# RobustFieldAutonomyLab/DRL_graph_exploration

Hardware: AMD Instinct MI355X
Metric: env-steps/sec (256 parallel envs, ~64-node graphs) (higher is better)
Workload: dtype f64; 1 GPU; configs[1]: 256 envs/GPU, 40x40 map (V=1600), 100 landmarks, belief update at ~59-node graphs (P=37.0 poses, L=22.2 landmarks, M=188 factors) from a device snapshot; envs_per_gpu=256, map_size=40, num_landmarks=100, parallelism=env-sharded x1

## Files before the change

### drl_graph_exploration_amd/csrc/drlgx_dev.h

```cpp
#pragma once
#include <hip/hip_runtime.h>
#include <stdint.h>

#include "../../include/drlgx.h"
#include "map_carve.h"

#define DRLGX_MT_N 624
#define DRLGX_MT_STRIDE 626
#define DRLGX_CNT_STRIDE 8
#define DRLGX_RED_STRIDE 8
#define DRLGX_PRIOR_STRIDE 16

enum { C_P = 0, C_L = 1, C_M = 2, C_STEP = 3, C_ISAM = 4, C_NEWP = 5, C_NEWL = 6, C_FLAG = 7 };
enum { R_UTR = 0, R_KNOWN = 1, R_EXPL = 2, R_UDET = 3, R_UWTR = 4, R_DIST = 5, R_OBS = 6, R_LATCH = 7 };

struct DrlgxState {
  drlgx_config cfg;
  int n_envs, n_inst, n_roll;
  int P_max, L_max, M_max, LG, V, Vu, rows, cols, A_max;
  int win;
  int disc_cells;
  int count_explored;
  double lo_free, lo_occ, lo_min, lo_max, occ_thresh;
  int bbox_noop;
// ... 76 lines not shown
#define DRLGX_KS_REF (*(const DrlgxState *)S_)
#define DRLGX_KS_ARG(S) ((DrlgxStateConst)(S).self_dev)

#define DRLGX_PROF(S, slot)                                                        \
  do {                                                                             \
    if ((S).prof && threadIdx.x == 0 && blockIdx.x == (S).prof_block) (S).prof[slot] = wall_clock64(); \
  } while (0)

__device__ __forceinline__ int drlgx_bid() {
  int b = blockIdx.x;
  asm volatile("" : "+v"(b));
  return __builtin_amdgcn_readfirstlane(b);
}

__device__ __forceinline__ int drlgx_tid() {
  int t = threadIdx.x;
  asm volatile("" : "+v"(t));
  return t;
}

struct LaunchSel {
  int base;
  int n;
  const uint8_t *active;
  const int32_t *n_act;
  int act_idx;
  int map_last_only = 0;
  int pcap = 0;
  int skip_map = 0;
  const unsigned char *simlog = nullptr;
  size_t simlog_roll = 0;
  int simlog_act = 0;
  int vm_from = -1;
  __host__ __device__ __forceinline__ int cap(int P_max) const { return pcap > 0 && pcap < P_max ? pcap : P_max; }
  __device__ __forceinline__ bool map_on(int i) const {
    return !(map_last_only && n_act) || act_idx == n_act[i] - 1;
  }
  __device__ __forceinline__ bool on(int i) const {
    if (active && !active[i]) return false;
    if (n_act && act_idx >= n_act[i]) return false;
    return true;
  }
};

struct Pose {
  double x, y, c, s;
};
struct P2 {
  double x, y;
};

__device__ __forceinline__ void rot_from_cos_sin(double c, double s, double &oc, double &os) {
  if (fabs(c * c + s * s - 1.0) > 1e-9) {
    double n = sqrt(c * c + s * s);
    c /= n;
    s /= n;
  }
  oc = c;
  os = s;
}
__device__ __forceinline__ Pose make_pose(double x, double y, double th) { return Pose{x, y, cos(th), sin(th)}; }
__device__ __forceinline__ double theta_of(const Pose &p) { return atan2(p.s, p.c); }
__device__ __forceinline__ Pose compose(const Pose &a, const Pose &b) {
  Pose r;
  rot_from_cos_sin(a.c * b.c - a.s * b.s, a.s * b.c + a.c * b.s, r.c, r.s);
  r.x = a.x + (a.c * b.x - a.s * b.y);
// ... 492 lines not shown
```

### drl_graph_exploration_amd/csrc/drlgx_engine.cpp

```cpp
#include <hip/hip_runtime.h>

#include <algorithm>
#include <chrono>
#include <cmath>
#include <cstdio>
#include <cstring>
#include <functional>
#include <string>
#include <unordered_map>
#include <cstdlib>
#include <vector>

#include "drlgx_dev.h"
#include "drlgx_fields.h"

#define HIPCHK(e, call)                                                                       \
  do {                                                                                        \
    hipError_t _r = (call);                                                                   \
    if (_r != hipSuccess) {                                                                   \
      (e)->last_error = std::string(#call) + ": " + hipGetErrorString(_r);                    \
      return DRLGX_E_HIP;                                                                     \
    }                                                                                         \
  } while (0)

// ... 39 lines not shown
  bool la_loop = true;
  double *fm2_sig = nullptr, *fm2_scratch = nullptr;
  int *fm2_iscratch = nullptr;
  int32_t *fm2_slot = nullptr;
  size_t fm2_sig_stride = 0, fm2_scratch_stride = 0;
  double *em_cov = nullptr;
  int32_t *em_nout = nullptr;
  int *em_flag = nullptr;
  int *og_flag = nullptr;
  double *tree_act = nullptr, *tree_cand_act = nullptr, *tree_cost = nullptr;
  int *tree_link = nullptr, *tree_leaf = nullptr, *tree_meta = nullptr;
  int32_t *tree_cand_env = nullptr, *tree_cand_n = nullptr;
  size_t tree_nodes_cap = 0, tree_sel_cap = 0, tree_cand_cap = 0;
  double sampler_max_nodes = 0.5, sampler_safe_distance = 0.0;
  int sampler_dubins = 0;
  int sampler_obstacles = 0;
  int env_obstacles = 0;
  double *follow_act = nullptr;
  int dubins_leaf_scoring = 0;
  uint8_t *tree_cand_core = nullptr;
  double *tree_cand_dist = nullptr;
  size_t tree_cand_steps_cap = 0, tree_cand_last = 0;
  bool tree_cand_last_steps = false;
  DrlgxDubins dubins = {};
  double *dub_end_x = nullptr, *dub_end_y = nullptr, *dub_v = nullptr, *dub_w = nullptr, *tree_pose = nullptr;
  int *dub_steps = nullptr;
  size_t dub_cap = 0, tree_pose_cap = 0;
  double dub_reach = 0.0;
  int dub_prefilter = 1;
  std::vector<double> dub_end_h, dub_v_h, dub_w_h;
  std::vector<int> dub_steps_h;
  int owed_slot = -1;
  bool restore_eager = false;
};

#define DRLGX_ENTER_OWING(e)                    \
  do {                                          \
    if (e) {                                    \
      (void)hipSetDevice((e)->device);          \
      state_sync(e);                            \
    }                                           \
  } while (0)
#define DRLGX_ENTER(e)                          \
  do {                                          \
    DRLGX_ENTER_OWING(e);                       \
    if (e) settle(e);                           \
  } while (0)

struct drlgx_engine;
static void state_sync(drlgx_engine *e);
static void settle(drlgx_engine *e);

namespace {

template <typename T>
int dev_alloc(drlgx_engine *e, T **out, size_t count) {
  void *p = nullptr;
  size_t bytes = std::max<size_t>(count * sizeof(T), 256);
  HIPCHK(e, hipMalloc(&p, bytes));
  HIPCHK(e, hipMemsetAsync(p, 0, bytes, e->stream));
  e->allocs.push_back(p);
  *out = reinterpret_cast<T *>(p);
  return DRLGX_OK;
}

template <typename T>
// ... 59 lines not shown
      cfg->max_actions < 1 || cfg->num_samples < 1)
    return DRLGX_E_INVALID;
  if (!(cfg->resolution >= 1)) {
    g_create_error = "resolution must be at least 1";
    return DRLGX_E_INVALID;
  }
  if (cfg->max_poses > 65535 || cfg->max_landmarks > 65535 || cfg->max_factors > 65534) return DRLGX_E_INVALID;
  if (!drlgx_slam_capacity_ok(cfg->max_poses, cfg->max_landmarks, cfg->max_factors)) return DRLGX_E_INVALID;
  const double cells = std::floor((cfg->map_max_x - cfg->map_min_x) / cfg->resolution) *
                       std::floor((cfg->map_max_y - cfg->map_min_y) / cfg->resolution);
  if (!(cells <= 65535.0) || !drlgx_graph_capacity_ok(cfg->max_poses, cfg->max_landmarks, (int)cells)) {
    g_create_error = "max_landmarks x max_poses (or the cell count of the map) too large for the LDS tables of the graph export";
    return DRLGX_E_INVALID;
  }
  if (kmap::MapCarve(cfg->max_poses, 1, (int)cells, false).bytes > kmap::kLdsBudget) {
    g_create_error = "map too large for the LDS tables of the map kernel";
    return DRLGX_E_INVALID;
  }
  return DRLGX_OK;
}

static bool env_flag(const char *name, bool dflt) {
  const char *v = getenv(name);
  if (!v) return dflt;
  return dflt ? v[0] != '0' : v[0] == '1';
}

static void read_env_switches(drlgx_engine *e) {
  e->by_capacity = env_flag("DRLGX_VARIANT_BY_CAPACITY", false);
  e->spin_sync = env_flag("DRLGX_SYNC_SPIN", true);
  e->la_presim = env_flag("DRLGX_LOOKAHEAD_PRESIM", true);
  e->la_loop = env_flag("DRLGX_LOOKAHEAD_LOOP", true);
  e->restore_eager = env_flag("DRLGX_RESTORE_EAGER", false);
}

static double p2l(double p) { return std::log(p / (1.0 - p)); }
static double l2p(double l) { return std::exp(l) / (1.0 + std::exp(l)); }

static int disc_cells_bound(double r) {
  const int n = 32;
  const double h = 0.5 / n, rr = r + h * 0.70710678118654752440 + 1e-9;
  const int k = (int)std::ceil(rr) + 1;
  int best = 0;
  for (int a = 0; a < n; ++a)
    for (int b = 0; b < n; ++b) {
      const double u = (a + 0.5) * h, v = (b + 0.5) * h;
      int cnt = 0;
      for (int i = -k; i <= k; ++i)
        for (int j = -k; j <= k; ++j)
          if ((i - u) * (i - u) + (j - v) * (j - v) <= rr * rr) ++cnt;
      best = std::max(best, cnt);
    }
  return best;
}

static int set_map_constants(drlgx_engine *e) {
  DrlgxState &S = e->S;
  const drlgx_config *cfg = &S.cfg;
  S.P_max = cfg->max_poses;
  S.L_max = cfg->max_landmarks;
  S.M_max = cfg->max_factors;
  S.LG = std::max(cfg->num_landmarks, 1);
  S.A_max = cfg->max_actions;
  S.cols = (int)std::floor((cfg->map_max_x - cfg->map_min_x) / cfg->resolution);
  S.rows = (int)std::floor((cfg->map_max_y - cfg->map_min_y) / cfg->resolution);
  S.V = S.rows * S.cols;
// ... 411 lines not shown
  DRLGX_ENTER_OWING(e);
  if (!e || (bytes > 0 && (!src_dev || !dst_host))) return DRLGX_E_INVALID;
  return status_fetch(e, src_dev, bytes, dst_host);
}

int drlgx_reset_host(drlgx_engine *e, int n, const int32_t *env_ids, const uint32_t *seeds, const double *start) {
  DRLGX_ENTER(e);
  if (!e || n <= 0 || n > e->S.n_envs || !env_ids || !seeds || !start) return DRLGX_E_INVALID;
  std::vector<uint8_t> mask(e->S.n_envs, 0);
  for (int i = 0; i < n; ++i) {
    if (env_ids[i] < 0 || env_ids[i] >= e->S.n_envs || mask[env_ids[i]]) return DRLGX_E_INVALID;
    mask[env_ids[i]] = 1;
  }
  HIPCHK(e, hipMemcpyAsync(e->stage_i32, env_ids, n * sizeof(int32_t), hipMemcpyHostToDevice, e->stream));
  HIPCHK(e, hipMemcpyAsync(e->stage_u32, seeds, n * sizeof(uint32_t), hipMemcpyHostToDevice, e->stream));
  HIPCHK(e, hipMemcpyAsync(e->stage_f64, start, n * 3 * sizeof(double), hipMemcpyHostToDevice, e->stream));
  HIPCHK(e, hipMemcpyAsync(e->stage_mask, mask.data(), e->S.n_envs, hipMemcpyHostToDevice, e->stream));
  HIPCHK(e, hipMemsetAsync(e->S.status, 0, sizeof(int), e->stream));
  drlgx_launch_reset(e->S, e->stream, n, e->stage_i32, e->stage_u32, e->stage_f64);
  for (int i = 0; i < n; ++i) e->pbound[env_ids[i]] = 1;
  LaunchSel sel{0, e->S.n_envs, e->stage_mask, nullptr, 0};
  drlgx_launch_slam(e->S, e->stream, sel, e->by_capacity ? e->S.P_max : 1);
  sel.pcap = max_bound(e);
  drlgx_launch_map(e->S, e->stream, sel, 0);
  int r = check_launch(e);
  if (r) return r;
  HIPCHK(e, hipStreamSynchronize(e->stream));
  return DRLGX_OK;
}

static void launch_belief_step(drlgx_engine *e, LaunchSel sel, const double *odom, int odom_stride, int n_measure, int pb, bool may_split,
                               bool obstacles = false) {
  const DrlgxState &S = e->S;
  sel.pcap = pb;
  if (drlgx_step_fusable(S, pb) && !e->per_stage && !obstacles) {
    ScopedTimer t(e, 5);
    const bool split = may_split && sel.n > e->n_cu && drlgx_map_two_per_cu(S, pb);
    sel.skip_map = split ? 1 : 0;
    drlgx_launch_step(S, e->stream, sel, odom, odom_stride, n_measure);
    if (split) {
      sel.skip_map = 0;
      drlgx_launch_map(S, e->stream, sel, 1);
    }
  } else if (drlgx_step_arrow_fusable(S) && !e->per_stage && !obstacles) {
    ScopedTimer t(e, 5);
    drlgx_launch_step_arrow(S, e->stream, sel, odom, odom_stride, n_measure);
  } else {
    {
      ScopedTimer t(e, 0);
      if (obstacles) drlgx_launch_sim_obs(S, e->stream, sel, odom, odom_stride);
      else drlgx_launch_sim(S, e->stream, sel, odom, odom_stride, n_measure);
    }
    {
      ScopedTimer t(e, 1);
      drlgx_launch_slam(S, e->stream, sel, pb);
    }
    {
      ScopedTimer t(e, 2);
      drlgx_launch_map(S, e->stream, sel, 1);
    }
  }
}

static bool env_obstacles_on(const drlgx_engine *e) { return e->env_obstacles && e->S.cfg.safe_distance > 0.0; }

int drlgx_step(drlgx_engine *e, const double *odom_dev, const uint8_t *active_dev) {
// ... 11 lines not shown
  return check_launch(e);
}

int drlgx_step_plan(drlgx_engine *e, const double *actions_dev, const int32_t *n_actions_dev, int action_index, int map_last_only) {
  DRLGX_ENTER(e);
  if (!e || !actions_dev || !n_actions_dev || action_index < 0 || action_index >= e->S.A_max) return DRLGX_E_INVALID;
  LaunchSel sel{0, e->S.n_envs, nullptr, n_actions_dev, action_index};
  sel.map_last_only = map_last_only ? 1 : 0;
  const int pb = std::min(max_bound(e) + 1, e->S.P_max);
  advance_pbound(e, 1);
  launch_belief_step(e, sel, actions_dev, e->S.A_max * 3, 2, pb, false, env_obstacles_on(e));
  return check_launch(e);
}

static void presimulate(drlgx_engine *e, LaunchSel &sel, const double *act, int n_measure, int max_n_actions) {
  const DrlgxState &S = e->S;
  const size_t entry = drlgx_simlog_entry_bytes(S), roll = entry * (size_t)S.A_max;
  if (!e->simlog_dev && dev_alloc(e, &e->simlog_dev, roll * (size_t)S.n_roll) != DRLGX_OK) {
    (void)hipGetLastError();
    e->last_error.clear();
    e->la_presim = false;
    return;
  }
  ScopedTimer t(e, 0);
  drlgx_launch_presim(S, e->stream, sel, act, S.A_max * 3, n_measure, max_n_actions, e->simlog_dev, roll, (int)entry);
  sel.simlog = e->simlog_dev;
  sel.simlog_roll = roll;
  sel.simlog_act = (int)entry;
}

static int launch_action_range(drlgx_engine *e, LaunchSel sel, const double *act, int n_measure, int pbe, int max_n_actions, bool partial,
                               bool presim) {
  const DrlgxState &S = e->S;
  int a_sw = 0;
  while (a_sw < max_n_actions && drlgx_step_fusable(S, std::min(pbe + a_sw + 1, S.P_max))) ++a_sw;
  const bool rest_loops = a_sw == max_n_actions || drlgx_step_arrow_fusable(S);
  if (!e->la_loop || e->per_stage || !(rest_loops || (partial && a_sw > 0))) return 0;
  if (presim && e->la_presim && rest_loops) presimulate(e, sel, act, n_measure, max_n_actions);
  ScopedTimer t(e, 5);
  if (a_sw > 0) {
    sel.act_idx = 0;
    sel.pcap = std::min(pbe + 1, S.P_max);
    drlgx_launch_step_loop(S, e->stream, sel, act, S.A_max * 3, n_measure, a_sw);
  }
  if (a_sw == max_n_actions || !rest_loops) return a_sw;
  sel.act_idx = a_sw;
  sel.pcap = std::min(pbe + a_sw + 1, S.P_max);
  drlgx_launch_step_arrow_loop(S, e->stream, sel, act, S.A_max * 3, n_measure, max_n_actions);
  return max_n_actions;
}

int drlgx_step_plans(drlgx_engine *e, const double *actions_dev, const int32_t *n_actions_dev, int max_n_actions, int map_last_only) {
  DRLGX_ENTER(e);
  if (!e || !actions_dev || !n_actions_dev || max_n_actions < 0 || max_n_actions > e->S.A_max) return DRLGX_E_INVALID;
  if (max_n_actions == 0) return DRLGX_OK;
  LaunchSel sel{0, e->S.n_envs, nullptr, n_actions_dev, 0};
  sel.map_last_only = map_last_only ? 1 : 0;
  const int a_begin = env_obstacles_on(e) ? 0 : launch_action_range(e, sel, actions_dev, 2, max_bound(e), max_n_actions, false, false);
  advance_pbound(e, a_begin);
  for (int a = a_begin; a < max_n_actions; ++a) {
    const int r = drlgx_step_plan(e, actions_dev, n_actions_dev, a, map_last_only);
    if (r) return r;
  }
  return check_launch(e);
}

// ... 58 lines not shown
  HIPCHK(e, hipMemsetAsync(e->S.status, 0, sizeof(int), e->stream));
  drlgx_launch_reset(e->S, e->stream, n, e->stage_i32, e->stage_u32, e->stage_f64, 0);
  for (int i = 0; i < n; ++i) e->pbound[env_ids[i]] = 1;
  int r = check_launch(e);
  if (r) return r;
  HIPCHK(e, hipStreamSynchronize(e->stream));
  return DRLGX_OK;
}
int drlgx_stage_move(drlgx_engine *e, const double *odom_dev, const uint8_t *active_dev) {
  DRLGX_ENTER(e);
  if (!e || !odom_dev) return DRLGX_E_INVALID;
  advance_pbound(e, 1);
  drlgx_launch_sim_stage(e->S, e->stream, LaunchSel{0, e->S.n_envs, active_dev, nullptr, 0}, odom_dev, 0, nullptr, nullptr, nullptr);
  return check_launch(e);
}
int drlgx_stage_measure(drlgx_engine *e, const uint8_t *active_dev, int32_t *keys_dev, double *bearing_range_dev, int32_t *count_dev) {
  DRLGX_ENTER(e);
  if (!e || !keys_dev || !bearing_range_dev || !count_dev) return DRLGX_E_INVALID;
  HIPCHK(e, hipMemsetAsync(count_dev, 0, sizeof(int32_t) * e->S.n_envs, e->stream));
  drlgx_launch_sim_stage(e->S, e->stream, LaunchSel{0, e->S.n_envs, active_dev, nullptr, 0}, nullptr, 1, keys_dev, bearing_range_dev,
                         count_dev);
  return check_launch(e);
}
int drlgx_stage_add_measurements(drlgx_engine *e, const uint8_t *active_dev, const int32_t *keys_dev, const double *bearing_range_dev,
                                 const int32_t *count_dev) {
  DRLGX_ENTER(e);
  if (!e || !keys_dev || !bearing_range_dev || !count_dev) return DRLGX_E_INVALID;
  drlgx_launch_add_measurements(e->S, e->stream, LaunchSel{0, e->S.n_envs, active_dev, nullptr, 0}, keys_dev, bearing_range_dev, count_dev);
  return check_launch(e);
}
int drlgx_stage_optimize(drlgx_engine *e, const uint8_t *active_dev) {
  DRLGX_ENTER(e);
  if (!e) return DRLGX_E_INVALID;
  drlgx_launch_slam(e->S, e->stream, LaunchSel{0, e->S.n_envs, active_dev, nullptr, 0}, max_bound(e));
  return check_launch(e);
}
int drlgx_stage_update_map(drlgx_engine *e, const uint8_t *active_dev, int rebuild) {
  DRLGX_ENTER(e);
  if (!e) return DRLGX_E_INVALID;
  drlgx_launch_map(e->S, e->stream, LaunchSel{0, e->S.n_envs, active_dev, nullptr, 0}, rebuild ? 1 : 0);
  return check_launch(e);
}

static const int kFm2Chunk = 128, kFm2MaxMeas = 256;
static int fm2_run(drlgx_engine *e, int n_cand, const int32_t *cand_env_dev, const double *actions_dev, const int32_t *n_actions_dev,
                   const uint8_t *core_dev, double *cov_out, int out_stride_poses, int32_t *n_out, bool chunk_out, const std::function<void(int, int)> &after) {
  const DrlgxState &S = e->S;
  if (!e->fm2_sig) {
    const size_t nmax = (size_t)3 * S.P_max + 2 * S.L_max;
    e->fm2_sig_stride = nmax * nmax;
    e->fm2_scratch_stride = drlgx_fm2_scratch_doubles(S, kFm2MaxMeas);
    int r;
    if ((r = dev_alloc(e, &e->fm2_sig, e->fm2_sig_stride * (size_t)S.n_envs))) return r;
    if ((r = dev_alloc(e, &e->fm2_scratch, e->fm2_scratch_stride * (size_t)kFm2Chunk))) return r;
    if ((r = dev_alloc(e, &e->fm2_iscratch, (size_t)2 * kFm2MaxMeas * kFm2Chunk))) return r;
    if ((r = dev_alloc(e, &e->fm2_slot, (size_t)S.n_envs))) return r;
    std::vector<int32_t> ident(S.n_envs);
    for (int i = 0; i < S.n_envs; ++i) ident[i] = i;
    HIPCHK(e, hipMemcpyAsync(e->fm2_slot, ident.data(), ident.size() * sizeof(int32_t), hipMemcpyHostToDevice, e->stream));
    HIPCHK(e, hipStreamSynchronize(e->stream));
  }
  drlgx_launch_fm2_prior(S, e->stream, nullptr, S.n_envs, e->fm2_sig, e->fm2_sig_stride, 3 * S.P_max + 2 * S.L_max);
  for (int c0 = 0; c0 < n_cand; c0 += kFm2Chunk) {
    const int nc = std::min(kFm2Chunk, n_cand - c0);
    drlgx_launch_fm2_update(S, e->stream, 0, nc, cand_env_dev + c0, e->fm2_slot, actions_dev + (size_t)c0 * S.A_max * 3, n_actions_dev + c0,
                            core_dev ? core_dev + (size_t)c0 * S.A_max : nullptr, e->fm2_sig, e->fm2_sig_stride, e->fm2_scratch, e->fm2_scratch_stride, e->fm2_iscratch, kFm2MaxMeas,
                            chunk_out ? cov_out : cov_out + (size_t)c0 * out_stride_poses * 9, out_stride_poses,
// ... 869 lines not shown
```

### drl_graph_exploration_amd/csrc/k_inc.hip

```cpp

#pragma once
#include <type_traits>
#include "k_slam_common.hip"
namespace kslam {
#pragma clang fp contract(on)

constexpr int IYS = 18;
constexpr int INF = 64;
constexpr int kStreamKB = 512;
constexpr int ISNT = 4;

__device__ __forceinline__ int *inc_meta(const DrlgxState &S, int inst) { return S.jc_meta + (size_t)inst * 4; }

__device__ __forceinline__ bool inc_precheck(const DrlgxState &S, int inst, int P_after, int tid, int *scratch, int meta0 = -1, int meta1 = 0,
                                             int isam = 0) {
  if (!S.jc) return false;
  const int *meta = inc_meta(S, inst);
  const int *cnt = S.cnt + (size_t)inst * DRLGX_CNT_STRIDE;
  if (meta0 < 0) {
    meta0 = meta[0];
    meta1 = meta[1];
    isam = cnt[C_ISAM];
  }
  if (meta0 != 1 || meta1 + 1 != P_after || P_after < 2) return false;
// ... 72 lines not shown
  x.fq = reinterpret_cast<double *>(take(32 * 8));
  x.recs = reinterpret_cast<double *>(take(INF * REC * 8));
  x.gs = reinterpret_cast<double *>(take(INEW * 12 * 8));
  x.vvec = reinterpret_cast<double *>(take(32 * 8));
  x.wks = reinterpret_cast<double *>(take(5 * 16 * IYS * 8));
  x.thp = reinterpret_cast<double *>(take((size_t)P * 4 * 8));
  x.thl = reinterpret_cast<double *>(take((size_t)x.Lcap * 2 * 8));
  x.dl = reinterpret_cast<double *>(take((size_t)ncap * 8));
  x.Dl = reinterpret_cast<double *>(take((size_t)P * 6 * 8));
  x.Y = reinterpret_cast<double *>(take((size_t)(x.n1p + 1) * IYS * 8));
  x.cwl = reinterpret_cast<double *>(smem_raw + off);
  const size_t fixed = ((plan_off + 15) & ~(size_t)15) + (off - off0);
  if (fixed > (size_t)lds_bytes) return false;
  lds_panel = fixed + (size_t)ncap * x.ldw * 8 <= (size_t)lds_bytes;
  const size_t pan = lds_panel ? (size_t)ncap * x.ldw * 8 : 0, yh = (size_t)(x.n1p + 1) * IYS * 8;
  x.Yh = x.cwl + pan / 8;
  x.wide = fixed + pan + yh <= (size_t)lds_bytes;
  x.snt = 0;
  if (!lds_panel && (3 * P + 1 + 15) / 16 > kDenseTiles) {
    x.yrows = x.a0 + 1;
    const size_t y_off = (size_t)(reinterpret_cast<unsigned char *>(x.Y) - smem_raw);
    const size_t avail = (size_t)lds_bytes - (((plan_off + 15) & ~(size_t)15) + (y_off - off0));
    for (int t = ISNT; t >= 1 && !x.snt; --t)
      if ((size_t)t * x.yrows * IYS * 8 + (size_t)max(0, t * t - 5) * 16 * IYS * 8 + (size_t)16 * t * 8 * 8 + 64 * 8 <= avail) x.snt = t;
    x.yt = x.Y;
    x.wim = x.yt + (size_t)x.snt * x.yrows * IYS;
    x.jt = x.wim + (size_t)max(0, x.snt * x.snt - 5) * 16 * IYS;
    x.svv = x.jt + (size_t)16 * x.snt * 8;
  }
  return true;
}

template <bool kLds, bool kSub>
__device__ __forceinline__ void inc_pre(const DrlgxState &S, const IncCtx &x, int tid, const double *odom3, SubBarrier sb) {
  const int ft = kSub ? tid - 64 : tid, fn = kSub ? kThreads - 64 : kThreads, lane = tid & 63;
  auto bar = [&]() {
    if constexpr (kSub) sb.sync(lane);
    else __syncthreads();
  };
  const int inst = x.inst, P = x.P, pn = x.pn, pp = x.pp, L0 = x.L0, n1 = x.n1, a0 = x.a0;
  double *gpan = S.jc + (size_t)inst * S.jc_stride;
  auto growp = [&](int q) -> double * { return gpan + (size_t)(q < 3 * P ? q : q + 3 * (S.P_max - P)) * S.jc_ld; };
  auto rowp = [&](int q) -> double * {
    if constexpr (kLds) return x.cwl + (size_t)q * x.ldw;
    else return gpan + (size_t)(q < 3 * P ? q : q + 3 * (S.P_max - P)) * S.jc_ld;
  };
  const double *th_pose = S.th_pose + (size_t)inst * S.P_max * 4;
  const double *th_lm = S.th_lm + (size_t)inst * S.L_max * 2;
  const double *d_pose = S.d_pose + (size_t)inst * S.P_max * 3;
  const double *d_lm = S.d_lm + (size_t)inst * S.L_max * 2;
  const double *jd = S.jd + (size_t)inst * S.P_max * 6;
  if (S.prof && blockIdx.x == S.prof_block && ft == 0) S.prof[0] = wall_clock64();
  if (ft < 4) x.ictl[ft] = 0;
  if (ft == fn - 1) {
    const double *t1 = th_pose + 4 * pp;
    Pose p1{t1[0], t1[1], t1[2], t1[3]}, p2, om;
    if constexpr (kSub) {
      om = make_pose(odom3[0], odom3[1], odom3[2]);
      const double *ep = S.est_pose + ((size_t)inst * S.P_max + pp) * 4;
      p2 = compose(Pose{ep[0], ep[1], ep[2], ep[3]}, om);
    } else {
      const double *t2 = th_pose + 4 * pn, *oo = S.odo + ((size_t)inst * S.P_max + pp) * 4;
      p2 = Pose{t2[0], t2[1], t2[2], t2[3]};
      om = Pose{oo[0], oo[1], oo[2], oo[3]};
    }
    double H1[9];
    const Pose hx = between(p1, p2, H1);
// ... 19 lines not shown
        const int q0 = qq, q1 = qq + rs, q2 = qq + 2 * rs, q3 = qq + 3 * rs;
        auto src = [&](int q) { const int c = min(q, nr - 1); return reinterpret_cast<const double2 *>(growp(c < 3 * pn ? c : c + 3))[cp]; };
        const double2 v0 = src(q0), v1 = src(q1), v2 = src(q2), v3 = src(q3);
        auto dst = [&](int q, const double2 &v) { if (q < nr) reinterpret_cast<double2 *>(rowp(q < 3 * pn ? q : q + 3))[cp] = v; };
        dst(q0, v0); dst(q1, v1); dst(q2, v2); dst(q3, v3);
      }
  }
  for (int e = ft; e < (x.n1p + 1 - n1) * IYS; e += fn) {
    x.Y[(size_t)n1 * IYS + e] = 0.0;
    if (x.wide) x.Yh[(size_t)n1 * IYS + e] = 0.0;
  }
  bar();
  if (S.prof && blockIdx.x == S.prof_block && ft == 0) S.prof[1] = wall_clock64();
  const double *fq = x.fq;
  {
    const double f00 = fq[0], f01 = fq[1], f02 = fq[2], f10 = fq[3], f11 = fq[4], f12 = fq[5], f20 = fq[6], f21 = fq[7], f22 = fq[8];
    for (int qq = ft; qq < n1 - 3; qq += fn) {
      const int q = qq < 3 * pn ? qq : qq + 3;
      double *r = rowp(q);
      const double t0 = r[0], t1 = r[1], t2 = r[2];
      r[0] = f00 * t0 + f01 * t1 + f02 * t2;
      r[1] = f10 * t0 + f11 * t1 + f12 * t2;
      r[2] = f20 * t0 + f21 * t1 + f22 * t2;
    }
  }
  bar();
  for (int e = ft; e < 3 * a0; e += fn) {
    const int r = e / a0, c = e - r * a0;
    double v = fq[3 * r] * rowp(3 * pp)[c] + fq[3 * r + 1] * rowp(3 * pp + 1)[c] + fq[3 * r + 2] * rowp(3 * pp + 2)[c];
    if (c == r) v += 1.0 / (c < 2 ? S.w_trans : S.w_rot);
    rowp(3 * pn + r)[c] = v;
  }
  if (ft < 3) x.dl[3 * pn + ft] = fq[3 * ft] * x.dl[3 * pp] + fq[3 * ft + 1] * x.dl[3 * pp + 1] + fq[3 * ft + 2] * x.dl[3 * pp + 2] + fq[9 + ft];
  if (S.prof && blockIdx.x == S.prof_block && ft == 0) S.prof[2] = wall_clock64();
}

template <bool kLds, int kSNT = ISNT>
__device__ __forceinline__ bool inc_post(const DrlgxState &S, const IncCtx &x, int L, int M, const SimBox &box, int tid,
                                         double *hand = nullptr, int hand_cap = 0) {
  const int lane = tid & 63, wave = tid >> 6, lc = lane & 15, lr = lane >> 4;
  const int inst = x.inst, P = x.P, pn = x.pn, L0 = x.L0, M0 = x.M0, n1 = x.n1, n1p = x.n1p, a0 = x.a0;
  int *meta = inc_meta(S, inst);
  const int nf = M - M0, nn = L - L0;
  const int n = 3 * P + 2 * L, a = 3 + 2 * L;
  int *fre = x.fre, *fnew = x.fnew, *fslot = x.fslot, *ictl = x.ictl;
  double *recs = x.recs, *gs = x.gs, *vvec = x.vvec, *wks = x.wks, *thp = x.thp, *thl = x.thl, *dl = x.dl, *Dl = x.Dl, *Y = x.Y;
  double *gpan = S.jc + (size_t)inst * S.jc_stride;
  auto growp = [&](int q) -> double * { return gpan + (size_t)(q < 3 * P ? q : q + 3 * (S.P_max - P)) * S.jc_ld; };
  auto rowp = [&](int q) -> double * {
    if constexpr (kLds) return x.cwl + (size_t)q * x.ldw;
    else return gpan + (size_t)(q < 3 * P ? q : q + 3 * (S.P_max - P)) * S.jc_ld;
  };
  int *cnt = S.cnt + (size_t)inst * DRLGX_CNT_STRIDE;
  double *d_pose = S.d_pose + (size_t)inst * S.P_max * 3;
  double *d_lm = S.d_lm + (size_t)inst * S.L_max * 2;
  double *jd = S.jd + (size_t)inst * S.P_max * 6;
  const bool feasible = nf >= 0 && nf <= INF && nn >= 0 && nn <= nf && L <= x.Lcap;
  const int *slot_src = box.br ? box.slot : S.meas_lm + (size_t)inst * S.M_max + M0;
  const double *br_src = box.br ? box.br : S.meas_br + ((size_t)inst * S.M_max + M0) * 2;
  const double *nl_src = box.br ? box.lm : S.th_lm + ((size_t)inst * S.L_max + L0) * 2;
  if (feasible && tid < 64) {
    const bool have = tid < nf;
    const int slot = have ? slot_src[tid] : -1;
    if (have) fslot[tid] = slot;
    bool bad = have && (slot < 0 || slot >= L);
    if (have && !box.br) bad |= S.meas_pose[(size_t)inst * S.M_max + M0 + tid] != pn;
    for (int t = 0; t < nf; ++t) {
      const int st = __builtin_amdgcn_readlane(slot, t);
      bad |= have && t < tid && st == slot;
    }
    const bool re = have && slot < L0, nw = have && slot >= L0;
    const unsigned long long mre = __ballot(re), mnw = __ballot(nw);
    if (re) fre[__popcll(mre & ((1ull << lane) - 1ull))] = tid;
    if (nw && !bad) fnew[slot - L0] = tid;
    if ((__ballot(bad) || __popcll(mnw) != nn) && lane == 0) ictl[2] = 1;
    if (lane == 0) ictl[0] = __popcll(mre);
  }
  for (int e = tid - 64; e >= 0 && e < 2 * nn && feasible; e += kThreads - 64) thl[2 * L0 + e] = nl_src[e];
  __syncthreads();
  if (!feasible || ictl[2]) {
    if (!kLds && tid == 0) meta[0] = 0;
    return false;
  }
  const int n_re = ictl[0];
  if (tid < nf) linearize_br(thp + 4 * pn, thl + 2 * fslot[tid], br_src[2 * tid], br_src[2 * tid + 1], recs + (size_t)REC * tid);
  __syncthreads();
  DRLGX_PROF(S, 35);
  const double Rb = S.cfg.bearing_noise * S.cfg.bearing_noise, Rr = S.cfg.range_noise * S.cfg.range_noise;
  const int ntr = n1p >> 4, ntc = (a0 + 15) >> 4;
  auto batch = [&](int b0, int nb, auto wide_tag) {
    constexpr bool kWide = decltype(wide_tag)::value;
    const int k = 2 * nb, kD = kWide ? k - 16 : 0;
    double *Yh = x.Yh;
    {
      constexpr int FS = kWide ? 16 : 8, RS = kThreads / FS;
      const int f = tid & (FS - 1);
      double j0 = 0, j1 = 0, j2 = 0, j3 = 0, j4 = 0, j5 = 0, l0c = 0, l1c = 0, l2c = 0, l3c = 0;
      int cl = 3;
      if (f < nb) {
        const int t = fre[b0 + f];
        const double *rc = recs + (size_t)REC * t;
        j0 = rc[0]; j1 = rc[1]; j2 = rc[2]; j3 = rc[3]; j4 = rc[4]; j5 = rc[5];
        l0c = rc[6]; l1c = rc[7]; l2c = rc[8]; l3c = rc[9];
        cl = 3 + 2 * fslot[t];
      }
      double *Yf = (kWide && f >= 8) ? Yh : Y;
      const int k0 = ks16(2 * (f & 7)), k1 = ks16(2 * (f & 7) + 1);
      for (int q0 = tid / FS; q0 < n1; q0 += 4 * RS) {
        double c0[4], c1[4], c2[4], l0[4], l1[4];
#pragma unroll
        for (int u = 0; u < 4; ++u) {
          const double *r = rowp(min(q0 + u * RS, n1 - 1));
          c0[u] = r[0]; c1[u] = r[1]; c2[u] = r[2]; l0[u] = r[cl]; l1[u] = r[cl + 1];
        }
#pragma unroll
        for (int u = 0; u < 4; ++u) {
          const int q = q0 + u * RS;
          if (q < n1) {
            Yf[(size_t)q * IYS + k0] = c0[u] * j0 + c1[u] * j1 + c2[u] * j2 + l0[u] * l0c + l1[u] * l1c;
            Yf[(size_t)q * IYS + k1] = c0[u] * j3 + c1[u] * j4 + c2[u] * j5 + l0[u] * l2c + l1[u] * l3c;
          }
        }
      }
    }
    __syncthreads();
    if (b0 == 0) DRLGX_PROF(S, 36);
    if (wave == 0) {
      auto tent = [&](int i, int j) -> double {
        const int t = fre[b0 + (i >> 1)], u = i & 1;
        const double *rc = recs + (size_t)REC * t;
        const double *Yj = (kWide && j >= 16) ? Yh : Y;
        const int col = ks16(j & 15);
        const double *yp = Yj + (size_t)(3 * pn) * IYS + col, *yl = Yj + (size_t)(3 * P + 2 * fslot[t]) * IYS + col;
        double sv = rc[3 * u] * yp[0] + rc[3 * u + 1] * yp[IYS] + rc[3 * u + 2] * yp[2 * IYS] + rc[6 + 2 * u] * yl[0] + rc[7 + 2 * u] * yl[IYS];
        if (i == j) sv += u ? Rr : Rb;
        return sv;
      };
      if (lane < (kWide ? 32 : 16)) {
        double v = 0.0;
        if (lane < k) {
          const int t = fre[b0 + (lane >> 1)], u = lane & 1;
// ... 568 lines not shown
    cnt[C_ISAM] = cnt[C_ISAM] + 1;
    cnt[C_NEWP] = P;
    cnt[C_NEWL] = L;
    if (ictl[1]) atomicMin(S.status, DRLGX_E_NUMERIC);
    if (S.inc_stats) atomicAdd(S.inc_stats, 1ull);
  }
  DRLGX_PROF(S, 7);
  return true;
}

__device__ __forceinline__ void panel_invalidate(const DrlgxState &S, int inst, int tid) {
  if (S.jc && tid == 0) {
    inc_meta(S, inst)[0] = 0;
    if (S.inc_stats) atomicAdd(S.inc_stats + 1, 1ull);
  }
}

#pragma clang fp contract(fast)

template <int kSNT>
__device__ __forceinline__ bool inc_stage(const DrlgxState &S, const LaunchSel &sel, int lds_bytes, size_t smem_off) {
  const int tid = drlgx_tid(), bi = drlgx_bid();
  if (!S.jc || !sel.on(bi)) return false;
  const int inst = sel.base + bi;
  const int *cnt = S.cnt + (size_t)inst * DRLGX_CNT_STRIDE;
  if (cnt[C_FLAG]) return false;
  const int P = cnt[C_P], L = cnt[C_L], M = cnt[C_M];
  extern __shared__ __attribute__((aligned(16))) unsigned char smem_raw[];
  if (!inc_precheck(S, inst, P, tid, reinterpret_cast<int *>(smem_raw + smem_off))) return false;
  IncCtx x;
  bool lds_panel = false;
  if (!inc_plan(S, inst, P, lds_bytes, smem_off, x, lds_panel, sel.cap(S.P_max))) return false;
  const SimBox nobox{nullptr, nullptr, nullptr};
  bool done;
  if (lds_panel) {
    inc_pre<true, false>(S, x, tid, nullptr, SubBarrier{nullptr, 0, 0});
    __syncthreads();
    done = inc_post<true, kSNT>(S, x, L, M, nobox, tid);
  } else {
    inc_pre<false, false>(S, x, tid, nullptr, SubBarrier{nullptr, 0, 0});
    __syncthreads();
    done = inc_post<false, kSNT>(S, x, L, M, nobox, tid);
  }
  if (!done) __syncthreads();
  return done;
}
#pragma clang fp contract(off)
}
```

### drl_graph_exploration_amd/csrc/k_slam_common.hip

```cpp
#pragma once
#include "k_sweep.hip"
#include "arrow_carve.h"
#include "slam_carve.h"
namespace kslam {
#pragma clang fp contract(fast)
constexpr int kLdsBudget = 160 * 1024;
static_assert(kFastTilesArrow == 8, "inc_plan (k_inc.hip) spells the reach of k_step_arrow out as 16 * 8");

constexpr int REC = 12;

#pragma clang fp contract(on)
__device__ __forceinline__ void linearize_br(const double *tp, const double *tl, double bm, double rm, double *rec) {
  Pose ps{tp[0], tp[1], tp[2], tp[3]};
  P2 lm{tl[0], tl[1]};
  const P2 d = transform_to(ps, lm);
  const double d2 = d.x * d.x + d.y * d.y, n = sqrt(d2);
  double sm, cm;
  sincos(bm, &sm, &cm);
  if (n > 1e-5) {
    const double in = 1.0 / n;
    const double c = d.x * in, s = d.y * in;
    const double a = -s * in, b = c * in;
    rec[0] = -a;
    rec[1] = -b;
    rec[2] = a * d.y - b * d.x;
    rec[3] = -c;
    rec[4] = -s;
    rec[5] = 0.0;
    rec[6] = a * ps.c - b * ps.s;
    rec[7] = a * ps.s + b * ps.c;
    rec[8] = ps.c * c - ps.s * s;
    rec[9] = ps.s * c + ps.c * s;
    rec[10] = atan2(-sm * c + cm * s, cm * c + sm * s);
    rec[11] = n - rm;
  } else {
    double Jx[6], Jl[4];
    (void)bearing_of<true>(ps, lm, Jx, Jl);
    const double rp = range_of<true>(ps, lm, Jx + 3, Jl + 2);
    for (int k = 0; k < 6; ++k) rec[k] = Jx[k];
    for (int k = 0; k < 4; ++k) rec[6 + k] = Jl[k];
    rec[10] = atan2(-sm, cm);
    rec[11] = rp - rm;
  }
}

__device__ __forceinline__ size_t up8(size_t b) { return (b + 7) & ~(size_t)7; }

#pragma clang fp contract(fast)
#define FOR_EACH_OBSERVING_POSE(mk, W, p)                                      \
  for (int _w = 0; _w < (W); ++_w)                                            \
    for (unsigned long long _m = (mk)[_w]; _m; _m &= _m - 1)                  \
      if (const int p = 64 * _w + __ffsll((long long)_m) - 1; true)

__device__ __forceinline__ void pose_block(const DrlgxState &S, int inst, const double *thp, const double *odo, const double *rec, const int *mstart,
                                           int i, int P, double wb, double wr, double *B, double *g, double *O) {
  const drlgx_config &cfg = S.cfg;
  for (int k = 0; k < 9; ++k) B[k] = 0.0;
  for (int k = 0; k < 3; ++k) g[k] = 0.0;
  const Pose ti{thp[4 * i], thp[4 * i + 1], thp[4 * i + 2], thp[4 * i + 3]};
  if (i == 0) {
    const double *pr = S.prior + (size_t)inst * DRLGX_PRIOR_STRIDE;
    const Pose h = between(Pose{pr[0], pr[1], pr[2], pr[3]}, ti, nullptr);
    const double e[3] = {h.x, h.y, theta_of(h)};
    const double J[9] = {h.c, h.s, 0, -h.s, h.c, 0, 0, 0, 1};
    const double *W = pr + 4;
    double WJ[9], We[3];
    for (int r = 0; r < 3; ++r) {
      for (int c = 0; c < 3; ++c) WJ[r * 3 + c] = W[r * 3] * J[c] + W[r * 3 + 1] * J[3 + c] + W[r * 3 + 2] * J[6 + c];
      We[r] = W[r * 3] * e[0] + W[r * 3 + 1] * e[1] + W[r * 3 + 2] * e[2];
    }
    for (int r = 0; r < 3; ++r) {
      for (int c = 0; c < 3; ++c) B[r * 3 + c] += J[r] * WJ[c] + J[3 + r] * WJ[3 + c] + J[6 + r] * WJ[6 + c];
      g[r] += J[r] * We[0] + J[3 + r] * We[1] + J[6 + r] * We[2];
    }
  }
  const double wo[3] = {1.0 / (cfg.translation_noise * cfg.translation_noise),
// ... 121 lines not shown
```

### drl_graph_exploration_amd/csrc/k_step.hip

```cpp
#include "drlgx_dev.h"

#include "k_sim.hip"
#include "k_sweep.hip"
#include "k_slam_common.hip"
#include "k_inc.hip"
#include "k_slam.hip"
#include "k_slam_arrow.hip"
#include "k_slam_host.hip"
#include "k_map.hip"
#include "k_em.hip"
#include "k_og.hip"

namespace kstep {

__host__ __device__ inline size_t sim_lds_bytes(int LG, int P_max) { return drlgx_sim_lds_bytes(LG, P_max); }

template <int FT>
__device__ __forceinline__ void step_once(const DrlgxState &S, const LaunchSel &sel, const double *odom, int odom_stride, int n_measure,
                                          int lds_bytes, int map_chunk) {
  static_assert(kslam::kThreads == kmap::kThreads, "the fused kernel runs both stages with one workgroup size");
  extern __shared__ __attribute__((aligned(16))) unsigned char step_smem[];
  const int tid = drlgx_tid();
  const int bi = drlgx_bid();
  if (S.prof && tid == 0 && bi < 448) S.prof[128 + 2 * bi] = wall_clock64();
// ... 23 lines not shown
      pan_L0 = mv.z;
      pan_M0 = mv.w;
    }
    const double *od = odom + (size_t)bi * odom_stride + (size_t)sel.act_idx * 3;
    od3[0] = od[0]; od3[1] = od[1]; od3[2] = od[2];
    if (spre.have) ksim::sim_preload(S, inst, tid, n_measure, spre);
    accepted = ksim::move_accepted(S, od3[0], od3[1], P0);
    inc_try = accepted && kslam::inc_precheck(S, inst, P0 + 1, tid, sub_cnt, meta0, meta1, isam);
    const int Lb = min(S.L_max, L0 + 48), Mb = min(S.M_max, M0 + 48);
    pre = accepted && !inc_try && (3 * (P0 + 1) + 1 + 15) / 16 <= kslam::kDenseTiles && kslam::SlamCtx::big_fits(sim_bytes, lds_bytes, P0 + 1, Lb, Mb);
    if (pre) ctx.setup<true>(S, step_smem, sim_bytes, lds_bytes, inst, P0 + 1, Lb, Mb);
  }
  if (tid == 0) {
    sub_cnt[0] = 0;
    sub_cnt[1] = -1;
  }
  __syncthreads();
  if (tid < 64) {
    uint32_t *l0 = reinterpret_cast<uint32_t *>(step_smem);
    uint32_t *l1 = l0 + DRLGX_MT_STRIDE;
    double *dyn = sim_dyn;
    if (sel.simlog)
      ksim::replay_step_body(S, sel, odom, odom_stride, tid, sub_cnt + 1);
    else
      ksim::sim_step_body(S, sel, odom, odom_stride, n_measure, l0, l1, dyn, tid, nullptr, nullptr, nullptr, true, sub_cnt + 1,
                          n_measure == 2 ? lmbox : nullptr, sel.on(bi) ? P0 : -1, L0, M0, spre);
  } else if (pre) {
    ctx.front<true>(S, tid, P0, L0, M0, P0, L0, isam + 1, false, od3, kslam::SubBarrier{sub_cnt, kslam::kThreads / 64 - 1, 0});
  } else if (inc_try) {
    kslam::IncCtx ix;
    bool inc_lds = false;
    if (kslam::inc_plan(S, sel.base + bi, P0 + 1, lds_bytes, sim_bytes, ix, inc_lds, pc, pan_L0, pan_M0)) {
      const kslam::SubBarrier sb{sub_cnt, kslam::kThreads / 64 - 1, 0};
      if (inc_lds) kslam::inc_pre<true, true>(S, ix, tid, od3, sb);
      else kslam::inc_pre<false, true>(S, ix, tid, od3, sb);
    }
  }
  __syncthreads();
  DRLGX_PROF(S, 32);
  if (accepted && tid >= 64 && !sel.simlog) {
    uint32_t *g = S.mt + (size_t)(sel.base + bi) * 2 * DRLGX_MT_STRIDE;
    const uint32_t *img = reinterpret_cast<const uint32_t *>(step_smem);
    for (int i = tid - 64; i < 2 * DRLGX_MT_STRIDE; i += kslam::kThreads - 64) g[i] = img[i];
  }
  const kmap::MapCarve map_carve(pc, map_chunk, S.V, false);
  const bool hand = map_carve.stage + 16 <= sim_bytes - 16;
  const double *lm_lds = nullptr;
  bool inc_done = false;
  if (inc_try) {
    kslam::IncCtx ix;
    bool inc_lds = false;
    if (kslam::inc_plan(S, sel.base + bi, P0 + 1, lds_bytes, sim_bytes, ix, inc_lds, pc, pan_L0, pan_M0)) {
      double *hp = hand ? reinterpret_cast<double *>(step_smem) : nullptr;
      inc_done = inc_lds ? kslam::inc_post<true, 0>(S, ix, sub_cnt[2], sub_cnt[3], box, tid, hp, pc)
                         : kslam::inc_post<false, 0>(S, ix, sub_cnt[2], sub_cnt[3], box, tid, hp, pc);
      if (inc_done) lm_lds = ix.thl;
      else __syncthreads();
    }
  }
  if (!inc_done)
    kslam::slam_finish<FT>(S, sel, lds_bytes, sim_bytes, ctx, pre, sub_cnt + 1, hand ? reinterpret_cast<double *>(step_smem) : nullptr, &lm_lds, box, pc);
  __syncthreads();
  const bool handed = hand && lm_lds != nullptr;
  if (sel.on(bi)) {
    const bool appended = sub_cnt[1] >= 0;
    lo.P = appended ? sub_cnt[1] : P0;
    lo.L = appended ? sub_cnt[2] : L0;
    lo.flag = appended ? 0 : 1;
  }
  const unsigned char *map_masks = step_smem + map_carve.mask;
  if (!handed || reinterpret_cast<const unsigned char *>(lm_lds + 2 * (size_t)S.L_max) > map_masks) lm_lds = nullptr;
  if (!sel.skip_map) kmap::map_body<false>(S, sel, 1, map_chunk, handed, lm_lds, lo);
  if (S.prof && tid == 0 && bi < 448) S.prof[129 + 2 * bi] = wall_clock64();
}

template <int FT>
__global__ __launch_bounds__(kslam::kThreads) void k_step(DrlgxState S, LaunchSel sel, const double *odom, int odom_stride,
                                                          int n_measure, int lds_bytes, int map_chunk) {
  step_once<FT>(S, sel, odom, odom_stride, n_measure, lds_bytes, map_chunk);
}

template <int FT>
__global__ __launch_bounds__(kslam::kThreads) void k_step_ref(DrlgxStateConst Sp, LaunchSel sel, const double *odom, int odom_stride,
                                                              int n_measure, int lds_bytes, int map_chunk) {
  if (__builtin_amdgcn_readfirstlane((int)threadIdx.x >> 6) == 0) drlgx_warm_state(Sp);
  step_once<FT>(*(const DrlgxState *)Sp, sel, odom, odom_stride, n_measure, lds_bytes, map_chunk);
}

// ... 98 lines not shown
```

Before: 4.051 million env-steps/sec.

## Pre-linearize landmark bearing-range Jacobians during the incremental-SLAM pre-phase

Splits bearing-range linearization into a Jacobian part and a measurement-error part. While the simulator waves run, the SLAM waves in inc_pre now compute the Jacobians for all existing landmarks into a scratch buffer. inc_post then copies those precomputed records and only linearizes new landmarks, with one wave computing the error terms while the others start the panel accumulation. This shortens the critical path after the sim phase, at the cost of extra linearization work for landmarks that may not be re-observed and more branching and scratch traffic.

After: 4.079 million env-steps/sec (median of 6 runs). About the same (+0.7%).

```diff
diff --git a/drl_graph_exploration_amd/csrc/drlgx_dev.h b/drl_graph_exploration_amd/csrc/drlgx_dev.h
--- a/drl_graph_exploration_amd/csrc/drlgx_dev.h
+++ b/drl_graph_exploration_amd/csrc/drlgx_dev.h
@@ -132,6 +132,7 @@
   size_t simlog_roll = 0;
   int simlog_act = 0;
   int vm_from = -1;
+  int inc_prelin = 0;
   __host__ __device__ __forceinline__ int cap(int P_max) const { return pcap > 0 && pcap < P_max ? pcap : P_max; }
   __device__ __forceinline__ bool map_on(int i) const {
     return !(map_last_only && n_act) || act_idx == n_act[i] - 1;
diff --git a/drl_graph_exploration_amd/csrc/drlgx_engine.cpp b/drl_graph_exploration_amd/csrc/drlgx_engine.cpp
--- a/drl_graph_exploration_amd/csrc/drlgx_engine.cpp
+++ b/drl_graph_exploration_amd/csrc/drlgx_engine.cpp
@@ -95,6 +95,7 @@
   std::vector<int> dub_steps_h;
   int owed_slot = -1;
   bool restore_eager = false;
+  bool inc_prelin = true;
 };
 
 #define DRLGX_ENTER_OWING(e)                    \
@@ -220,6 +221,7 @@
   e->la_presim = env_flag("DRLGX_LOOKAHEAD_PRESIM", true);
   e->la_loop = env_flag("DRLGX_LOOKAHEAD_LOOP", true);
   e->restore_eager = env_flag("DRLGX_RESTORE_EAGER", false);
+  e->inc_prelin = env_flag("DRLGX_INC_PRELIN", true);
 }
 
 static double p2l(double p) { return std::log(p / (1.0 - p)); }
@@ -697,6 +699,7 @@
 static void launch_belief_step(drlgx_engine *e, LaunchSel sel, const double *odom, int odom_stride, int n_measure, int pb, bool may_split,
                                bool obstacles = false) {
   const DrlgxState &S = e->S;
+  sel.inc_prelin = e->inc_prelin ? 1 : 0;
   sel.pcap = pb;
   if (drlgx_step_fusable(S, pb) && !e->per_stage && !obstacles) {
     ScopedTimer t(e, 5);
@@ -774,6 +777,7 @@
 static int launch_action_range(drlgx_engine *e, LaunchSel sel, const double *act, int n_measure, int pbe, int max_n_actions, bool partial,
                                bool presim) {
   const DrlgxState &S = e->S;
+  sel.inc_prelin = e->inc_prelin ? 1 : 0;
   int a_sw = 0;
   while (a_sw < max_n_actions && drlgx_step_fusable(S, std::min(pbe + a_sw + 1, S.P_max))) ++a_sw;
   const bool rest_loops = a_sw == max_n_actions || drlgx_step_arrow_fusable(S);
@@ -898,7 +902,9 @@
 int drlgx_stage_optimize(drlgx_engine *e, const uint8_t *active_dev) {
   DRLGX_ENTER(e);
   if (!e) return DRLGX_E_INVALID;
-  drlgx_launch_slam(e->S, e->stream, LaunchSel{0, e->S.n_envs, active_dev, nullptr, 0}, max_bound(e));
+  LaunchSel sel{0, e->S.n_envs, active_dev, nullptr, 0};
+  sel.inc_prelin = e->inc_prelin ? 1 : 0;
+  drlgx_launch_slam(e->S, e->stream, sel, max_bound(e));
   return check_launch(e);
 }
 int drlgx_stage_update_map(drlgx_engine *e, const uint8_t *active_dev, int rebuild) {
diff --git a/drl_graph_exploration_amd/csrc/k_inc.hip b/drl_graph_exploration_amd/csrc/k_inc.hip
--- a/drl_graph_exploration_amd/csrc/k_inc.hip
+++ b/drl_graph_exploration_amd/csrc/k_inc.hip
@@ -128,7 +128,7 @@
 }
 
 template <bool kLds, bool kSub>
-__device__ __forceinline__ void inc_pre(const DrlgxState &S, const IncCtx &x, int tid, const double *odom3, SubBarrier sb) {
+__device__ __forceinline__ void inc_pre(const DrlgxState &S, const IncCtx &x, int tid, const double *odom3, SubBarrier sb, bool prelin) {
   const int ft = kSub ? tid - 64 : tid, fn = kSub ? kThreads - 64 : kThreads, lane = tid & 63;
   auto bar = [&]() {
     if constexpr (kSub) sb.sync(lane);
@@ -214,11 +214,13 @@
     rowp(3 * pn + r)[c] = v;
   }
   if (ft < 3) x.dl[3 * pn + ft] = fq[3 * ft] * x.dl[3 * pp] + fq[3 * ft + 1] * x.dl[3 * pp + 1] + fq[3 * ft + 2] * x.dl[3 * pp + 2] + fq[9 + ft];
+  if (prelin)
+    for (int j = ft; j < L0; j += fn) linearize_br_jac(x.thp + 4 * pn, x.thl + 2 * j, x.Y + (size_t)REC * j);
   if (S.prof && blockIdx.x == S.prof_block && ft == 0) S.prof[2] = wall_clock64();
 }
 
 template <bool kLds, int kSNT = ISNT>
-__device__ __forceinline__ bool inc_post(const DrlgxState &S, const IncCtx &x, int L, int M, const SimBox &box, int tid,
+__device__ __forceinline__ bool inc_post(const DrlgxState &S, const IncCtx &x, int L, int M, const SimBox &box, int tid, bool prelin,
                                          double *hand = nullptr, int hand_cap = 0) {
   const int lane = tid & 63, wave = tid >> 6, lc = lane & 15, lr = lane >> 4;
   const int inst = x.inst, P = x.P, pn = x.pn, L0 = x.L0, M0 = x.M0, n1 = x.n1, n1p = x.n1p, a0 = x.a0;
@@ -265,7 +267,16 @@
     return false;
   }
   const int n_re = ictl[0];
-  if (tid < nf) linearize_br(thp + 4 * pn, thl + 2 * fslot[tid], br_src[2 * tid], br_src[2 * tid + 1], recs + (size_t)REC * tid);
+  if (prelin) {
+    for (int e = tid; e < REC * n_re; e += kThreads) {
+      const int i = e / REC, t = fre[i];
+      recs[(size_t)REC * t + (e - REC * i)] = Y[(size_t)REC * fslot[t] + (e - REC * i)];
+    }
+    const int t = kThreads - 1 - tid;
+    if (t < nf && fslot[t] >= L0) linearize_br(thp + 4 * pn, thl + 2 * fslot[t], br_src[2 * t], br_src[2 * t + 1], recs + (size_t)REC * t);
+  } else if (tid < nf) {
+    linearize_br(thp + 4 * pn, thl + 2 * fslot[tid], br_src[2 * tid], br_src[2 * tid + 1], recs + (size_t)REC * tid);
+  }
   __syncthreads();
   DRLGX_PROF(S, 35);
   const double Rb = S.cfg.bearing_noise * S.cfg.bearing_noise, Rr = S.cfg.range_noise * S.cfg.range_noise;
@@ -274,8 +285,15 @@
     constexpr bool kWide = decltype(wide_tag)::value;
     const int k = 2 * nb, kD = kWide ? k - 16 : 0;
     double *Yh = x.Yh;
-    {
-      constexpr int FS = kWide ? 16 : 8, RS = kThreads / FS;
+    const bool spare = prelin && b0 == 0;
+    if (spare && wave == 0) {
+      if (lane < n_re) {
+        const int t = fre[lane];
+        linearize_br_err(recs + (size_t)REC * t, br_src[2 * t], br_src[2 * t + 1]);
+      }
+    } else {
+      constexpr int FS = kWide ? 16 : 8;
+      const int RS = (spare ? kThreads - 64 : kThreads) / FS, rt = spare ? tid - 64 : tid;
       const int f = tid & (FS - 1);
       double j0 = 0, j1 = 0, j2 = 0, j3 = 0, j4 = 0, j5 = 0, l0c = 0, l1c = 0, l2c = 0, l3c = 0;
       int cl = 3;
@@ -288,7 +306,7 @@
       }
       double *Yf = (kWide && f >= 8) ? Yh : Y;
       const int k0 = ks16(2 * (f & 7)), k1 = ks16(2 * (f & 7) + 1);
-      for (int q0 = tid / FS; q0 < n1; q0 += 4 * RS) {
+      for (int q0 = rt / FS; q0 < n1; q0 += 4 * RS) {
         double c0[4], c1[4], c2[4], l0[4], l1[4];
 #pragma unroll
         for (int u = 0; u < 4; ++u) {
@@ -923,15 +941,16 @@
   bool lds_panel = false;
   if (!inc_plan(S, inst, P, lds_bytes, smem_off, x, lds_panel, sel.cap(S.P_max))) return false;
   const SimBox nobox{nullptr, nullptr, nullptr};
+  const bool prelin = kSNT == 0 && sel.inc_prelin != 0;
   bool done;
   if (lds_panel) {
-    inc_pre<true, false>(S, x, tid, nullptr, SubBarrier{nullptr, 0, 0});
-    __syncthreads();
-    done = inc_post<true, kSNT>(S, x, L, M, nobox, tid);
+    inc_pre<true, false>(S, x, tid, nullptr, SubBarrier{nullptr, 0, 0}, prelin);
+    __syncthreads();
+    done = inc_post<true, kSNT>(S, x, L, M, nobox, tid, prelin);
   } else {
-    inc_pre<false, false>(S, x, tid, nullptr, SubBarrier{nullptr, 0, 0});
-    __syncthreads();
-    done = inc_post<false, kSNT>(S, x, L, M, nobox, tid);
+    inc_pre<false, false>(S, x, tid, nullptr, SubBarrier{nullptr, 0, 0}, prelin);
+    __syncthreads();
+    done = inc_post<false, kSNT>(S, x, L, M, nobox, tid, prelin);
   }
   if (!done) __syncthreads();
   return done;
diff --git a/drl_graph_exploration_amd/csrc/k_slam_common.hip b/drl_graph_exploration_amd/csrc/k_slam_common.hip
--- a/drl_graph_exploration_amd/csrc/k_slam_common.hip
+++ b/drl_graph_exploration_amd/csrc/k_slam_common.hip
@@ -10,13 +10,11 @@
 constexpr int REC = 12;
 
 #pragma clang fp contract(on)
-__device__ __forceinline__ void linearize_br(const double *tp, const double *tl, double bm, double rm, double *rec) {
+__device__ __forceinline__ void linearize_br_jac(const double *tp, const double *tl, double *rec) {
   Pose ps{tp[0], tp[1], tp[2], tp[3]};
   P2 lm{tl[0], tl[1]};
   const P2 d = transform_to(ps, lm);
   const double d2 = d.x * d.x + d.y * d.y, n = sqrt(d2);
-  double sm, cm;
-  sincos(bm, &sm, &cm);
   if (n > 1e-5) {
     const double in = 1.0 / n;
     const double c = d.x * in, s = d.y * in;
@@ -31,17 +29,32 @@
     rec[7] = a * ps.s + b * ps.c;
     rec[8] = ps.c * c - ps.s * s;
     rec[9] = ps.s * c + ps.c * s;
-    rec[10] = atan2(-sm * c + cm * s, cm * c + sm * s);
-    rec[11] = n - rm;
+    rec[11] = n;
   } else {
     double Jx[6], Jl[4];
     (void)bearing_of<true>(ps, lm, Jx, Jl);
     const double rp = range_of<true>(ps, lm, Jx + 3, Jl + 2);
     for (int k = 0; k < 6; ++k) rec[k] = Jx[k];
     for (int k = 0; k < 4; ++k) rec[6 + k] = Jl[k];
+    rec[11] = rp;
+  }
+  rec[10] = n;
+}
+__device__ __forceinline__ void linearize_br_err(double *rec, double bm, double rm) {
+  const double n = rec[10], rp = rec[11];
+  double sm, cm;
+  sincos(bm, &sm, &cm);
+  if (n > 1e-5) {
+    const double c = -rec[3], s = -rec[4];
+    rec[10] = atan2(-sm * c + cm * s, cm * c + sm * s);
+  } else {
     rec[10] = atan2(-sm, cm);
-    rec[11] = rp - rm;
-  }
+  }
+  rec[11] = rp - rm;
+}
+__device__ __forceinline__ void linearize_br(const double *tp, const double *tl, double bm, double rm, double *rec) {
+  linearize_br_jac(tp, tl, rec);
+  linearize_br_err(rec, bm, rm);
 }
 
 __device__ __forceinline__ size_t up8(size_t b) { return (b + 7) & ~(size_t)7; }
diff --git a/drl_graph_exploration_amd/csrc/k_step.hip b/drl_graph_exploration_amd/csrc/k_step.hip
--- a/drl_graph_exploration_amd/csrc/k_step.hip
+++ b/drl_graph_exploration_amd/csrc/k_step.hip
@@ -79,8 +79,8 @@
     bool inc_lds = false;
     if (kslam::inc_plan(S, sel.base + bi, P0 + 1, lds_bytes, sim_bytes, ix, inc_lds, pc, pan_L0, pan_M0)) {
       const kslam::SubBarrier sb{sub_cnt, kslam::kThreads / 64 - 1, 0};
-      if (inc_lds) kslam::inc_pre<true, true>(S, ix, tid, od3, sb);
-      else kslam::inc_pre<false, true>(S, ix, tid, od3, sb);
+      if (inc_lds) kslam::inc_pre<true, true>(S, ix, tid, od3, sb, sel.inc_prelin != 0);
+      else kslam::inc_pre<false, true>(S, ix, tid, od3, sb, sel.inc_prelin != 0);
     }
   }
   __syncthreads();
@@ -99,8 +99,8 @@
     bool inc_lds = false;
     if (kslam::inc_plan(S, sel.base + bi, P0 + 1, lds_bytes, sim_bytes, ix, inc_lds, pc, pan_L0, pan_M0)) {
       double *hp = hand ? reinterpret_cast<double *>(step_smem) : nullptr;
-      inc_done = inc_lds ? kslam::inc_post<true, 0>(S, ix, sub_cnt[2], sub_cnt[3], box, tid, hp, pc)
-                         : kslam::inc_post<false, 0>(S, ix, sub_cnt[2], sub_cnt[3], box, tid, hp, pc);
+      inc_done = inc_lds ? kslam::inc_post<true, 0>(S, ix, sub_cnt[2], sub_cnt[3], box, tid, sel.inc_prelin != 0, hp, pc)
+                         : kslam::inc_post<false, 0>(S, ix, sub_cnt[2], sub_cnt[3], box, tid, sel.inc_prelin != 0, hp, pc);
       if (inc_done) lm_lds = ix.thl;
       else __syncthreads();
     }
```
